# voxel-tracer/ag-pathtracer

Measured on AMD Instinct MI355X. Metric: Mrays/sec (primary+secondary) at 1080p/64spp, higher is better.
Workload: dtype f32; 1 GPU; BASELINE configs[2]: Sponza-class closed atrium, 258672 tris / 37 primitives / 35 Disney materials, 1920x1080, 64 spp, PathTracer MaxDepth=5, NEE+MIS; triangles=258672, spp=64

## Files before the change

### ag-pathtracer_amd/csrc/agpt_api.hip

```cpp
#include <hip/hip_runtime.h>

#include <algorithm>
#include <cmath>
#include <cstdio>
#include <cstdlib>
#include <cstring>
#include <memory>
#include <string>
#include <vector>

#include "../../include/agpt.h"
#include "agpt_adaptive.h"
#include "agpt_bvh_device.h"
#include "agpt_denoise.h"
#include "agpt_host_scene.hpp"
#include "agpt_kernels.h"
#include "agpt_update.h"

#ifndef AGPT_FAST_STACK
#define AGPT_FAST_STACK 23
#endif
#ifndef AGPT_FAST_BLOCKS_PER_CU
#define AGPT_FAST_BLOCKS_PER_CU 5
#endif


namespace {

thread_local std::string g_error;

int fail(int code, const std::string& msg) {
    g_error = msg;
    return code;
}

}
namespace agpt {
int report_error(int code, const std::string& msg) { return fail(code, msg); }
}
namespace {

#define HIP_TRY(expr)                                                                                   \
    do {                                                                                                \
        hipError_t e_ = (expr);                                                                         \
        if (e_ != hipSuccess)                                                                           \
            return fail(AGPT_ERR_DEVICE, std::string(#expr) + ": " + hipGetErrorString(e_));           \
    } while (0)
// ... 28 lines not shown
    }
    void release() {
        if (p) (void)hipFree(p);
        p = nullptr;
        n = 0;
    }
};

}

#define AGPT_POOL_BUFFERS(X)                                                                                                  \
    X(float4, ext_o) X(float4, ext_d) X(float4, sh_o) X(float4, sh_d) X(float4, mis_o) X(float4, mis_d) X(float4, beta4)      \
    X(float4, L4) X(float4, fac4) X(float4, c1) X(float4, c2) X(DevHit, hit) X(DevHit, mis_hit) X(uint32_t, occluded)          \
    X(uint32_t, mis_ok)

struct agpt_ctx {
    int device = 0;
    hipStream_t stream = nullptr;
    int num_cus = 256;
    hipEvent_t ev[4] = {nullptr, nullptr, nullptr, nullptr};
    hipStream_t aux_stream[2] = {nullptr, nullptr};
    hipEvent_t aux_ev[3] = {nullptr, nullptr, nullptr};
    int multi_stream = 0;
    size_t pool_paths = 0;
#define X(T, name) DevBuf<T> name;
    AGPT_POOL_BUFFERS(X)
#undef X
    DevBuf<uint32_t> q[2][AGPT_NQUEUES];
    DevBuf<uint32_t> qcounts;
    DevBuf<uint32_t> work;
    DevBuf<DevCounters> counters;
    uint32_t* host_pinned = nullptr;
    int blocks_per_cu = 4;
    int shade_blocks_per_cu = 8;
    int fast_blocks_per_cu = AGPT_FAST_BLOCKS_PER_CU;
    DevBuf<uint32_t> spill;
    DevBuf<unsigned long long> cand_mask;
    DevBuf<uint32_t> cand_chunks;
    DevBuf<uint32_t> adapt_masks, adapt_blocks, adapt_list, adapt_words;
    DevBuf<float4> denoise_state;
    int refill = AGPT_REFILL;
    int refill_any = AGPT_REFILL_ANY;
    bool mis_closest = false;
    bool force_generic = false;
    std::vector<hipEvent_t> tev;
    size_t tev_used = 0;
// ... 70 lines not shown
}

static int trace_grid(const agpt_ctx* c) { return c->num_cus * c->blocks_per_cu; }
static int fast_grid(const agpt_ctx* c) { return c->num_cus * c->fast_blocks_per_cu; }

static bool use_fast_trace(const agpt_ctx* c, const DevScene& sc, int count) {
    return count != 1 && sc.n_prims <= 64 * AGPT_MAX_CHUNKS && !c->force_generic;
}

#define AGPT_SMALL_BATCH (48ull << 20)

struct TraceLaunch {
    hipStream_t stream;
    const uint32_t* queue;
    const uint32_t* count_ptr;
    uint32_t count_imm;
    uint32_t* work_head;
    const float4 *ro, *rd;
    DevHit* hits;
    uint32_t* occ;
    int count;
    bool small_batch;
    bool recast;
};

template <int MODE, bool COUNT, bool SPILL, bool PEEK>
static void launch_trace_fast(agpt_ctx* c, const DevScene& sc, const TraceLaunch& t) {
    const dim3 block(AGPT_BLOCK), g(fast_grid(c));
    const int refill = MODE == 0 ? c->refill : c->refill_any;
    if (sc.n_prims <= 64) {
        float4* ro_w = MODE == 0 && t.recast ? const_cast<float4*>(t.ro) : nullptr;
        float4* rd_w = MODE == 0 && t.recast ? const_cast<float4*>(t.rd) : nullptr;
        hipLaunchKernelGGL((k_trace_fast<MODE, AGPT_FAST_STACK, false, COUNT, SPILL, PEEK>), g, block, 0, t.stream, sc, t.queue, t.count_ptr,
                           t.count_imm, t.work_head, t.ro, t.rd, t.hits, t.occ, c->counters.p, refill, 0u, c->spill.p,
                           (const unsigned long long*)nullptr, (const uint32_t*)nullptr, ro_w, rd_w, (const float4*)c->beta4.p, c->L4.p);
        return;
    }
    const uint32_t stride = (uint32_t)c->pool_paths;
    if (c->cand_chunks.n < c->pool_paths || c->cand_mask.n < (size_t)((sc.n_prims + 63) / 64) * c->pool_paths) {
        c->note(hipErrorOutOfMemory);
        return;
    }
    hipLaunchKernelGGL((k_candidates<MODE>), dim3(c->num_cus * 8), block, 0, t.stream, sc, t.queue, t.count_ptr, t.count_imm, t.ro, t.rd,
                       c->cand_mask.p, c->cand_chunks.p, stride);
    hipLaunchKernelGGL((k_trace_fast<MODE, AGPT_FAST_STACK, true, COUNT, SPILL, PEEK>), g, block, 0, t.stream, sc, t.queue, t.count_ptr,
                       t.count_imm, t.work_head, t.ro, t.rd, t.hits, t.occ, c->counters.p, refill, stride, c->spill.p,
                       (const unsigned long long*)c->cand_mask.p, (const uint32_t*)c->cand_chunks.p, (float4*)nullptr, (float4*)nullptr,
                       (const float4*)nullptr, (float4*)nullptr);
}

template <bool ANY, bool COUNT, int DEPTH>
static void launch_trace_generic(agpt_ctx* c, int grid, const DevScene& sc, const TraceLaunch& t) {
    hipLaunchKernelGGL((k_trace<ANY, COUNT, DEPTH>), dim3(grid), dim3(AGPT_BLOCK), 0, t.stream, sc, t.queue, t.count_ptr, t.count_imm,
                       t.work_head, t.ro, t.rd, t.hits, t.occ, c->counters.p);
}

template <int MODE>
static void launch_trace(agpt_ctx* c, const DevScene& sc, const TraceLaunch& t) {
// ... 58 lines not shown

extern "C" {

const char* agpt_last_error(void) { return g_error.c_str(); }
int agpt_version(void) { return 1; }

int agpt_init(int device, agpt_ctx** out) {
    if (!out) return fail(AGPT_ERR_INVALID, "agpt_init: out is NULL");
    int n = 0;
    hipError_t e = hipGetDeviceCount(&n);
    if (e != hipSuccess || n == 0)
        return fail(AGPT_ERR_DEVICE, "agpt_init: no HIP device (the MI355X path has no CPU fallback)");
    if (device < 0 || device >= n) return fail(AGPT_ERR_INVALID, "agpt_init: bad device index");
    HIP_TRY(hipSetDevice(device));
    std::unique_ptr<agpt_ctx> c(new agpt_ctx());
    c->device = device;
    hipDeviceProp_t prop;
    HIP_TRY(hipGetDeviceProperties(&prop, device));
    c->num_cus = prop.multiProcessorCount > 0 ? prop.multiProcessorCount : 256;
    for (auto& ev : c->ev) HIP_TRY(hipEventCreate(&ev));
    for (auto& st : c->aux_stream) HIP_TRY(hipStreamCreateWithFlags(&st, hipStreamNonBlocking));
    for (auto& ev : c->aux_ev) HIP_TRY(hipEventCreateWithFlags(&ev, hipEventDisableTiming));
    if (const char* ms = getenv("AGPT_MULTI_STREAM")) c->multi_stream = atoi(ms);
    HIP_TRY(hipHostMalloc((void**)&c->host_pinned, 2 * AGPT_NQUEUES * AGPT_QSTRIDE * sizeof(uint32_t)));
    const char* fg = getenv("AGPT_FORCE_GENERIC");
    c->force_generic = fg && fg[0] == '1';
    if (const char* mc = getenv("AGPT_MIS_CLOSEST")) c->mis_closest = mc[0] == '1';
    if (const char* bp = getenv("AGPT_BLOCKS_PER_CU")) c->fast_blocks_per_cu = std::max(1, atoi(bp));
    if (const char* sb = getenv("AGPT_SHADE_BLOCKS_PER_CU")) c->shade_blocks_per_cu = std::min(64, std::max(1, atoi(sb)));
    if (const char* rf = getenv("AGPT_REFILL")) c->refill = std::min(64, std::max(1, atoi(rf)));
    if (const char* rf = getenv("AGPT_REFILL_ANY")) c->refill_any = std::min(64, std::max(1, atoi(rf)));
    *out = c.release();
    return AGPT_OK;
}

int agpt_set_stream(agpt_ctx* c, void* s) {
    if (!c) return fail(AGPT_ERR_INVALID, "agpt_set_stream: ctx is NULL");
    c->stream = (hipStream_t)s;
    return AGPT_OK;
}

void agpt_destroy(agpt_ctx* c) {
    if (!c) return;
    (void)hipSetDevice(c->device);
    (void)hipDeviceSynchronize();
    if (c->host_pinned) (void)hipHostFree(c->host_pinned);
    for (auto& ev : c->tev) (void)hipEventDestroy(ev);
    for (auto& ev : c->ev)
        if (ev) (void)hipEventDestroy(ev);
    for (auto& ev : c->aux_ev)
        if (ev) (void)hipEventDestroy(ev);
    for (auto& st : c->aux_stream)
        if (st) (void)hipStreamDestroy(st);
    delete c;
}

int agpt_scene_create(agpt_ctx* c, agpt_scene** out) {
    if (!c || !out) return fail(AGPT_ERR_INVALID, "agpt_scene_create: NULL argument");
    agpt_scene* s = new agpt_scene();
    s->ctx = c;
    *out = s;
    return AGPT_OK;
}

void agpt_scene_destroy(agpt_scene* s) {
    if (!s) return;
    (void)hipSetDevice(s->ctx->device);
    (void)hipDeviceSynchronize();
    delete s;
}

int agpt_scene_add_material(agpt_scene* s, int type, const float color[3], float roughness, float metallic) {
    if (!s || !color) return fail(AGPT_ERR_INVALID, "agpt_scene_add_material: NULL argument");
    if (type < AGPT_MAT_DISNEY || type > AGPT_MAT_DIFFUSE_ONLY) return fail(AGPT_ERR_INVALID, "unknown material type");
// ... 636 lines not shown
    HIP_TRY(hipStreamSynchronize(c->stream));
    return AGPT_OK;
}

#define X(T, name) +sizeof(T)
constexpr size_t AGPT_BYTES_PER_PATH = (0 AGPT_POOL_BUFFERS(X)) + 2 * AGPT_NQUEUES * sizeof(uint32_t);
#undef X
static_assert(AGPT_BYTES_PER_PATH == 256, "11 float4 arrays + 2 hit arrays (16 B) + 2 flag words + 10 queue words");
static size_t candidate_bytes_per_path(int n_prims) { return n_prims > 64 ? 4 + 8 * (size_t)((n_prims + 63) / 64) : 0; }
static int ensure_pool(agpt_ctx* c, size_t paths, int n_prims) {
    int rc;
    paths = std::max(paths, c->pool_paths);
    if (n_prims > 64) {
        if ((rc = c->cand_chunks.ensure(paths))) return rc;
        if ((rc = c->cand_mask.ensure(paths * (size_t)((n_prims + 63) / 64)))) return rc;
    }
#define X(T, name) \
    if ((rc = c->name.ensure(paths))) return rc;
    AGPT_POOL_BUFFERS(X)
#undef X
    for (int i = 0; i < 2; i++)
        for (int j = 0; j < AGPT_NQUEUES; j++)
            if ((rc = c->q[i][j].ensure(paths))) return rc;
    if ((rc = c->qcounts.ensure(2 * AGPT_NQUEUES * AGPT_QSTRIDE))) return rc;
    if ((rc = c->work.ensure(4096))) return rc;
    if ((rc = c->counters.ensure(1))) return rc;
    c->pool_paths = paths;
    return AGPT_OK;
}

static int fit_pool(agpt_ctx* c, const agpt_scene* s, size_t unit, uint64_t& count) {
    if (unit * (size_t)count > c->pool_paths) {
        size_t free_b = 0, total_b = 0;
        if (hipMemGetInfo(&free_b, &total_b) == hipSuccess) {
            const size_t per_path = AGPT_BYTES_PER_PATH + candidate_bytes_per_path(s->dev.n_prims);
            const size_t avail = free_b + c->pool_paths * per_path;
            const size_t fit = (size_t)((double)avail * 0.9) / per_path;
            while (count > 1 && unit * (size_t)count > fit) count = (count + 1) / 2;
        }
    }
    int rc = ensure_pool(c, unit * (size_t)count, s->dev.n_prims);
    while (rc == AGPT_ERR_NOMEM && count > 1) {
        release_pool(c);
        count = (count + 1) / 2;
        rc = ensure_pool(c, unit * (size_t)count, s->dev.n_prims);
    }
    return rc;
// ... 25 lines not shown
    run.count = enable_counters == 2 ? 2 : (enable_counters != 0 ? 1 : 0);
    run.mis_mode = use_fast_trace(c, s->dev, run.count) && !c->mis_closest;
    run.timing = timing;
    run.shade.fast = s->shading_arith == AGPT_SHADING_FAST;
    run.shade.textured = s->textured;
    run.shade.mapped = s->mapped;
    run.shade.sampled = s->sampled;
    run.shade.normal = s->normal;
    run.shade.lds_tables = shade_tables_fit_lds(s->dev);
    run.shade.env = !s->envs.empty();
    c->tev_used = 0;
    c->tev_kind.clear();
    HIP_TRY(hipMemsetAsync(c->counters.p, 0, sizeof(DevCounters), c->stream));
    HIP_TRY(hipEventRecord(c->ev[0], c->stream));
    return AGPT_OK;
}

static void set_wavefront_consts(RenderConsts& rc, const WavefrontRun& run, int max_depth, bool trace_all_rays) {
    rc.max_depth = max_depth;
    rc.mis_mode = run.mis_mode ? 1 : 0;
    rc.answer_rays = (run.mis_mode && !trace_all_rays) ? 1 : 0;
}

static int run_wavefront(agpt_ctx* c, agpt_scene* s, const RenderConsts& rcn, WavefrontRun& run) {
    const int count = run.count;
    const PathBuffers& pb = run.pb;
    Queues* const q = run.q;
    const int shade_grid = c->num_cus * c->shade_blocks_per_cu;
    const bool small_batch = (unsigned long long)rcn.NP * (unsigned long long)rcn.S < AGPT_SMALL_BATCH;
    const bool recast = !getenv("AGPT_NO_RECAST");
    const bool side = (c->multi_stream == 2 || (c->multi_stream == 1 && small_batch)) && use_fast_trace(c, s->dev, count) &&
                      s->dev.max_depth <= AGPT_FAST_STACK && s->dev.n_prims <= 64;
    const hipStream_t main_stream = c->stream, mis_stream = side ? c->aux_stream[0] : main_stream,
                      shadow_stream = side ? c->aux_stream[1] : main_stream;
    int cur = 0;
    const int planned = rcn.max_depth + 2;
    for (int it = 0;; it++) {
        if (it >= planned) {
            uint32_t* slot = c->host_pinned + (it & 1) * (AGPT_NQUEUES * AGPT_QSTRIDE);
            HIP_TRY(hipMemcpyAsync(slot, q[cur].counts, (4 * AGPT_QSTRIDE + 1) * sizeof(uint32_t), hipMemcpyDeviceToHost, main_stream));
            HIP_TRY(hipEventRecord(c->ev[2 + (it & 1)], main_stream));
            if (it > planned) {
                const uint32_t* seen = c->host_pinned + ((it - 1) & 1) * (AGPT_NQUEUES * AGPT_QSTRIDE);
                HIP_TRY(hipEventSynchronize(c->ev[2 + ((it - 1) & 1)]));
                if (seen[0] == 0 && seen[4 * AGPT_QSTRIDE] == 0) break;
            }
            if (it > 4096) return fail(AGPT_ERR_LIMIT, "agpt: path did not terminate");
        }
        const int nxt = cur ^ 1;
        HIP_TRY(hipMemsetAsync(q[nxt].counts, 0, AGPT_NQUEUES * AGPT_QSTRIDE * sizeof(uint32_t), main_stream));
        HIP_TRY(hipMemsetAsync(c->work.p, 0, 4 * AGPT_FRONTIERS * AGPT_QSTRIDE * sizeof(uint32_t), main_stream));
        uint32_t* const heads[4] = {c->work.p, c->work.p + AGPT_FRONTIERS * AGPT_QSTRIDE, c->work.p + 2 * AGPT_FRONTIERS * AGPT_QSTRIDE,
                                    c->work.p + 3 * AGPT_FRONTIERS * AGPT_QSTRIDE};
        const TraceLaunch ext{main_stream, q[cur].ext, &QCOUNT(q[cur], 1), 0, heads[0], pb.ext_o, pb.ext_d, pb.hit, nullptr,
                              count, small_batch, recast};
        const TraceLaunch mis{mis_stream, q[cur].mis, &QCOUNT(q[cur], 2), 0, heads[1], pb.mis_o, pb.mis_d,
                              run.mis_mode ? nullptr : pb.mis_hit, run.mis_mode ? pb.mis_ok : nullptr, count, small_batch, false};
        const TraceLaunch shadow{shadow_stream, q[cur].shadow, &QCOUNT(q[cur], 3), 0, heads[2], pb.sh_o, pb.sh_d, nullptr, pb.occluded,
                                 count, small_batch, false};
        auto trace_ext = [&]() { launch_trace_timed<0>(c, run.timing, 0, s->dev, ext); };
        auto trace_mis = [&]() {
            if (run.mis_mode) launch_trace_timed<2>(c, run.timing, 1, s->dev, mis);
            else launch_trace_timed<0>(c, run.timing, 1, s->dev, mis);
        };
        auto trace_shadow = [&]() { launch_trace_timed<1>(c, run.timing, 2, s->dev, shadow); };
        if (side) {
            HIP_TRY(hipEventRecord(c->aux_ev[0], main_stream));
            HIP_TRY(hipStreamWaitEvent(mis_stream, c->aux_ev[0], 0));
            HIP_TRY(hipStreamWaitEvent(shadow_stream, c->aux_ev[0], 0));
            trace_mis();
            HIP_TRY(hipEventRecord(c->aux_ev[1], mis_stream));
            trace_shadow();
            HIP_TRY(hipEventRecord(c->aux_ev[2], shadow_stream));
            trace_ext();
            HIP_TRY(hipStreamWaitEvent(main_stream, c->aux_ev[1], 0));
            HIP_TRY(hipStreamWaitEvent(main_stream, c->aux_ev[2], 0));
        } else {
            trace_ext();
            trace_mis();
            trace_shadow();
        }
        agpt::launch_shading(main_stream, run.shade, shade_grid, c->num_cus * 8, s->dev, rcn, pb, q[cur], q[nxt], c->counters.p, heads[3]);
        cur = nxt;
        run.iterations++;
        run.launches += 3;
    }
    return AGPT_OK;
}

static void read_counters(const DevCounters& d, agpt_stats* st) {
    st->closest_rays = d.closest_rays;
    st->anyhit_rays = d.anyhit_rays;
    st->interior_visits = d.interior;
    st->root_tests = d.roots;
    st->tri_tests = d.tris;
    st->shaded_vertices = d.shaded;
    st->outliers = d.outliers;
    st->samples = d.samples;
    st->answered_rays = d.answered;
}

static int end_wavefront(agpt_ctx* c) {
    HIP_TRY(hipEventRecord(c->ev[1], c->stream));
    HIP_TRY(hipGetLastError());
    HIP_TRY(c->take_deferred());
    return AGPT_OK;
}

static int fill_stats(agpt_ctx* c, const WavefrontRun& run, uint64_t samples, agpt_stats* stats) {
    if (!stats) return AGPT_OK;
// ... 211 lines not shown
int agpt_render(agpt_scene* s, const agpt_render_params* rp, float* accum_dev, agpt_stats* stats) {
    if (!s || !rp || !accum_dev) return fail(AGPT_ERR_INVALID, "agpt_render: NULL argument");
    if (!s->committed || !s->has_camera) return fail(AGPT_ERR_INVALID, "agpt_render: scene not committed or camera not set");
    int rc;
    if ((rc = check_tile("agpt_render", rp)) || (rc = check_depth("agpt_render", rp->max_depth))) return rc;
    if (rp->spp_count < 0) return fail(AGPT_ERR_INVALID, "agpt_render: bad sample range");
    agpt_ctx* c = s->ctx;
    HIP_TRY(hipSetDevice(c->device));
    uint32_t rows;
    if ((rc = tile_rows("agpt_render", rp, rows))) return rc;
    if (rows == 0) return AGPT_OK;
    const uint32_t NP = (uint32_t)rp->w * rows;
    uint64_t batch = std::min<uint64_t>(samples_per_batch(rp, NP), (uint64_t)std::max(1, rp->spp_count));
    if ((uint64_t)NP * batch > 0x7FFFFFFFull) return fail(AGPT_ERR_LIMIT, "agpt_render: batch too large");
    if ((rc = fit_pool(c, s, NP, batch))) return rc;
    const int S = (int)batch;
    s->dev.cam = s->cam;

    WavefrontRun run;
    if ((rc = begin_wavefront(c, s, rp->enable_counters, rp->enable_timing != 0 && stats != nullptr, run))) return rc;
    RenderConsts rcn = tile_consts(rp, NP);
    rcn.seed_base = rp->seed_base;
    set_wavefront_consts(rcn, run, rp->max_depth, rp->trace_all_rays != 0);
    for (int s0 = rp->spp_begin; s0 < rp->spp_begin + rp->spp_count; s0 += S) {
        rcn.s0 = s0;
        rcn.S = std::min(S, rp->spp_begin + rp->spp_count - s0);
        const uint32_t total = NP * (uint32_t)rcn.S;
        hipLaunchKernelGGL(k_generate, dim3((total + AGPT_BLOCK - 1) / AGPT_BLOCK), dim3(AGPT_BLOCK), 0, c->stream, s->dev, rcn, run.pb,
                           run.q[0]);
        if ((rc = run_wavefront(c, s, rcn, run))) return rc;
        hipLaunchKernelGGL(k_accumulate, dim3((NP + AGPT_BLOCK - 1) / AGPT_BLOCK), dim3(AGPT_BLOCK), 0, c->stream, rcn, run.pb,
                           (float4*)accum_dev, c->counters.p);
    }
    if ((rc = end_wavefront(c))) return rc;
    return fill_stats(c, run, (uint64_t)NP * (uint64_t)rp->spp_count, stats);
}

int agpt_render_adaptive(agpt_scene* s, const agpt_render_params* rp, const agpt_adaptive_params* ap, float* accum_dev,
                         float* moment2_dev, agpt_stats* stats, agpt_adaptive_stats* astats) {
    if (!s || !rp || !ap || !accum_dev || !moment2_dev) return fail(AGPT_ERR_INVALID, "agpt_render_adaptive: NULL argument");
    if (!s->committed || !s->has_camera) return fail(AGPT_ERR_INVALID, "agpt_render_adaptive: scene not committed or camera not set");
    int rc;
    if ((rc = check_tile("agpt_render_adaptive", rp)) || (rc = check_depth("agpt_render_adaptive", rp->max_depth))) return rc;
    if (rp->spp_begin != 0 || rp->spp_count != 0)
        return fail(AGPT_ERR_INVALID, "agpt_render_adaptive: spp_begin and spp_count must be 0 (the counts are in accum.w)");
    const int step = ap->step_spp, min_spp = ap->min_spp, max_spp = ap->max_spp;
    if (step < 1 || min_spp < 2 || min_spp > max_spp || max_spp > (1 << 24) || min_spp % step != 0 || max_spp % step != 0 ||
        !(ap->abs_floor >= 0.f) || ap->rel_error != ap->rel_error)
        return fail(AGPT_ERR_INVALID, "agpt_render_adaptive: need 1 <= step_spp, 2 <= min_spp <= max_spp <= 2^24, both multiples of "
                                      "step_spp, abs_floor >= 0, rel_error not NaN");
    if (astats) std::memset(astats, 0, sizeof(*astats));
    agpt_ctx* c = s->ctx;
    HIP_TRY(hipSetDevice(c->device));
    uint32_t rows;
    if ((rc = tile_rows("agpt_render_adaptive", rp, rows))) return rc;
// ... 496 lines not shown
```

### ag-pathtracer_amd/csrc/agpt_kernels.h

```cpp
#pragma once

#include "agpt_shade.h"
#include "agpt_trace.h"

#include "agpt_wavefront.h"

template <bool ANY, bool COUNT, int DEPTH>
__global__ void __launch_bounds__(AGPT_BLOCK)
k_trace(DevScene sc, const uint32_t* __restrict__ queue, const uint32_t* __restrict__ count_ptr, uint32_t count_imm,
        uint32_t* __restrict__ work_head, const float4* __restrict__ ray_o, const float4* __restrict__ ray_d,
        DevHit* __restrict__ hits, uint32_t* __restrict__ occluded, DevCounters* __restrict__ counters) {
    __shared__ uint32_t s_stack[DEPTH * AGPT_BLOCK];
    uint32_t* stack = s_stack + threadIdx.x;
    const int lane = threadIdx.x & 63;
    const uint32_t count = count_ptr ? *count_ptr : count_imm;
    TraceCounters cnt;
    cnt.interior = 0;
    cnt.tris = 0;
    cnt.roots = 0;
    cnt.last_mesh = 0;
    for (;;) {
        uint32_t base = 0;
        if (lane == 0) base = atomicAdd(work_head, (uint32_t)AGPT_CHUNK);
        base = __shfl(base, 0);
// ... 20 lines not shown
            atomicAdd(&counters->interior, (unsigned long long)cnt.interior);
            atomicAdd(&counters->tris, (unsigned long long)cnt.tris);
            atomicAdd(&counters->roots, (unsigned long long)cnt.roots);
        }
    }
    if (threadIdx.x == 0 && blockIdx.x == 0) {
        if (ANY)
            atomicAdd(&counters->anyhit_rays, (unsigned long long)count);
        else
            atomicAdd(&counters->closest_rays, (unsigned long long)count);
    }
}

#define AGPT_REFILL 20
#define AGPT_REFILL_ANY 40
#define AGPT_RING 128

#ifndef AGPT_TRACE_WAVES
#define AGPT_TRACE_WAVES 1
#endif
template <int MODE, int DEPTH, bool LIST, bool COUNT, bool SPILL, bool PEEK>
__global__ void __launch_bounds__(AGPT_BLOCK, AGPT_TRACE_WAVES)
k_trace_fast(DevScene sc, const uint32_t* __restrict__ queue, const uint32_t* __restrict__ count_ptr, uint32_t count_imm,
             uint32_t* __restrict__ work_head, const float4* __restrict__ ray_o, const float4* __restrict__ ray_d,
             DevHit* __restrict__ hits, uint32_t* __restrict__ occluded, DevCounters* __restrict__ counters, int refill,
             uint32_t cand_stride, uint32_t* __restrict__ spill, const unsigned long long* __restrict__ cand_mask,
             const uint32_t* __restrict__ cand_chunks, float4* ray_o_w, float4* ray_d_w, const float4* path_beta4, float4* path_L4) {
    constexpr bool ANY = MODE != 0;
    constexpr bool MIS = MODE == 2;
    constexpr int BLOCK = AGPT_BLOCK;
    constexpr bool PRIM_LDS = !LIST;
    __shared__ uint32_t s_stack[DEPTH * BLOCK];
    __shared__ float4 s_prim[PRIM_LDS ? 2 * 64 : 2];
    uint32_t* stack = s_stack + threadIdx.x;
    uint32_t* spill_col = SPILL ? spill + (size_t)blockIdx.x * BLOCK + threadIdx.x : nullptr;
    const size_t spill_stride = (size_t)gridDim.x * BLOCK;
    auto stack_push = [&](int k, uint32_t v) {
        if (!SPILL || k < DEPTH)
            stack[k * BLOCK] = v;
        else
            spill_col[(size_t)(k - DEPTH) * spill_stride] = v;
    };
    auto stack_at = [&](int k) -> uint32_t {
        if (!SPILL || k < DEPTH) return stack[k * BLOCK];
        return spill_col[(size_t)(k - DEPTH) * spill_stride];
    };
    const int lane = threadIdx.x & 63;
// ... 820 lines not shown
```

### ag-pathtracer_amd/csrc/agpt_shade_kernels.h

```cpp
#pragma once

#include "agpt_shade.h"
#include "agpt_trace.h"
#include "agpt_wavefront.h"

#ifndef AGPT_SHADE_TEXTURED
#define AGPT_SHADE_TEXTURED 0
#endif
#if AGPT_SHADE_TEXTURED == 4 && AGPT_SHADE_FAST
#define AGPT_SHADE_KNAME(n) n##_normal_fast
#elif AGPT_SHADE_TEXTURED == 4
#define AGPT_SHADE_KNAME(n) n##_normal
#elif AGPT_SHADE_TEXTURED == 3 && AGPT_SHADE_FAST
#define AGPT_SHADE_KNAME(n) n##_sampled_fast
#elif AGPT_SHADE_TEXTURED == 3
#define AGPT_SHADE_KNAME(n) n##_sampled
#elif AGPT_SHADE_TEXTURED == 2 && AGPT_SHADE_FAST
#define AGPT_SHADE_KNAME(n) n##_mapped_fast
#elif AGPT_SHADE_TEXTURED == 2
#define AGPT_SHADE_KNAME(n) n##_mapped
#elif AGPT_SHADE_TEXTURED && AGPT_SHADE_FAST
#define AGPT_SHADE_KNAME(n) n##_textured_fast
#elif AGPT_SHADE_TEXTURED
#define AGPT_SHADE_KNAME(n) n##_textured
// ... 411 lines not shown
    l4.x = L.x; l4.y = L.y; l4.z = L.z; l4.w = __uint_as_float(rng);
    pb.L4[pid] = l4;
    SCK(6);
    return bits;
}

#ifndef SHADE_GRAB
#define SHADE_GRAB 2
#endif
#ifndef SHADE_U
#define SHADE_U 4
#endif

#ifndef AGPT_SHADE_WAVES
#define AGPT_SHADE_WAVES 3
#endif
#define AGPT_SHADE_LDS_PRIMS 256
#define AGPT_SHADE_LDS_MATERIALS 128
#define AGPT_SHADE_LDS_LIGHTS 64
template <bool LDS_TABLES, bool ENV>
__global__ void __launch_bounds__(AGPT_BLOCK, AGPT_SHADE_WAVES)
AGPT_SHADE_KNAME(k_shade)(DevScene sc_in, RenderConsts rc, PathBuffers pb, Queues qin, Queues qout, DevCounters* __restrict__ counters,
        uint32_t* __restrict__ tile_heads) {
    __shared__ DevPrim s_tab_prims[LDS_TABLES ? AGPT_SHADE_LDS_PRIMS : 1];
    __shared__ DevMaterial s_tab_materials[LDS_TABLES ? AGPT_SHADE_LDS_MATERIALS : 1];
    __shared__ DevLight s_tab_lights[LDS_TABLES ? AGPT_SHADE_LDS_LIGHTS : 1];
#if AGPT_SHADE_TEXTURED
    constexpr int n_tab_halves = AGPT_SHADE_TEXTURED >= 2 ? 2 : 1;
    __shared__ int32_t s_tab_material_texture[LDS_TABLES ? n_tab_halves * AGPT_SHADE_LDS_MATERIALS : 1];
#endif
    if (blockIdx.x * (AGPT_BLOCK / 64) * 64u * SHADE_U >= QCOUNT(qin, 0) && blockIdx.x > 0) return;
    DevScene sc = sc_in;
    if (LDS_TABLES) {
        auto copy_words = [&](void* dst, const void* src, int n_bytes) {
            uint32_t* d = (uint32_t*)dst;
            const uint32_t* g = (const uint32_t*)src;
            for (int i = threadIdx.x; i < n_bytes / 4; i += AGPT_BLOCK) d[i] = g[i];
        };
        copy_words(s_tab_prims, sc_in.prims, sc_in.n_prims * (int)sizeof(DevPrim));
        copy_words(s_tab_materials, sc_in.materials, sc_in.n_materials * (int)sizeof(DevMaterial));
        copy_words(s_tab_lights, sc_in.lights, sc_in.n_lights * (int)sizeof(DevLight));
        sc.prims = s_tab_prims;
        sc.materials = s_tab_materials;
        sc.lights = s_tab_lights;
#if AGPT_SHADE_TEXTURED
        copy_words(s_tab_material_texture, sc_in.material_texture, n_tab_halves * sc_in.n_materials * (int)sizeof(int32_t));
        sc.material_texture = s_tab_material_texture;
#endif
        __syncthreads();
    }
    __shared__ uint32_t s_pid[SHADE_U][AGPT_BLOCK];
    __shared__ uint32_t s_bits[SHADE_U][AGPT_BLOCK];
    const uint32_t n_active = QCOUNT(qin, 0);
    const int tid = threadIdx.x, lane = tid & 63;
    const unsigned long long lt_mask = (1ull << lane) - 1ull;
    uint32_t shaded = 0, mis_answered = 0;
#ifdef AGPT_SHADE_CLOCK
    unsigned long long sck_acc[8] = {0, 0, 0, 0, 0, 0, 0, 0};
    unsigned long long sck_last = __builtin_amdgcn_s_memtime();
    const unsigned long long sck_begin = sck_last;
#endif
    const uint32_t wtile = 64u * SHADE_U;
    const uint32_t n_wtiles = (n_active + wtile - 1) / wtile;
    uint32_t seg = blockIdx.x & (AGPT_FRONTIERS - 1u), segs_left = AGPT_FRONTIERS;
    const uint32_t seg_tiles = (n_wtiles + AGPT_FRONTIERS - 1u) / AGPT_FRONTIERS;
    uint32_t t_next = 0, t_end = 0;
    auto next_tile = [&](uint32_t& t) -> bool {
        if (t_next < t_end) {
            t = t_next++;
            return true;
// ... 95 lines not shown
        const float4 c1_4 = pb.c1[pid], c2_4 = pb.c2[pid];
        const uint32_t flags = __float_as_uint(b4.w);
        const v3 Ld = pending_light_sample(sc, rc, pb, pid, flags, was_occluded, was_mis_ok, c1_4, c2_4, f4);
        const float lightPdf = sh_rcp(sc.n_lights);
        const v3 L = V3(l4.x, l4.y, l4.z) + V3(b4.x, b4.y, b4.z) * sh_div3(Ld, lightPdf);
        l4.x = L.x; l4.y = L.y; l4.z = L.z;
        pb.L4[pid] = l4;
    }
}
#endif

namespace agpt {
using ShadeLaunch = void(hipStream_t stream, int grid, bool lds_tables, bool env, const DevScene& sc, const RenderConsts& rc,
                         const PathBuffers& pb, const Queues& qin, const Queues& qout, DevCounters* counters, uint32_t* tile_heads);
using ResolveLaunch = void(hipStream_t stream, int grid, const DevScene& sc, const RenderConsts& rc, const PathBuffers& pb, const Queues& qin);
ShadeLaunch launch_shade, launch_shade_fast, launch_shade_textured, launch_shade_textured_fast, launch_shade_mapped, launch_shade_mapped_fast,
    launch_shade_sampled, launch_shade_sampled_fast, launch_shade_normal, launch_shade_normal_fast;
ResolveLaunch launch_resolve_pending, launch_resolve_pending_fast;

void AGPT_SHADE_KNAME(launch_shade)(hipStream_t stream, int grid, bool lds_tables, bool env, const DevScene& sc, const RenderConsts& rc,
                                    const PathBuffers& pb, const Queues& qin, const Queues& qout, DevCounters* counters,
                                    uint32_t* tile_heads) {
    const dim3 g(grid), b(AGPT_BLOCK);
    if (lds_tables && env)
        hipLaunchKernelGGL((AGPT_SHADE_KNAME(k_shade)<true, true>), g, b, 0, stream, sc, rc, pb, qin, qout, counters, tile_heads);
    else if (lds_tables)
        hipLaunchKernelGGL((AGPT_SHADE_KNAME(k_shade)<true, false>), g, b, 0, stream, sc, rc, pb, qin, qout, counters, tile_heads);
    else if (env)
        hipLaunchKernelGGL((AGPT_SHADE_KNAME(k_shade)<false, true>), g, b, 0, stream, sc, rc, pb, qin, qout, counters, tile_heads);
    else
        hipLaunchKernelGGL((AGPT_SHADE_KNAME(k_shade)<false, false>), g, b, 0, stream, sc, rc, pb, qin, qout, counters, tile_heads);
}
#if !AGPT_SHADE_TEXTURED
void AGPT_SHADE_KNAME(launch_resolve_pending)(hipStream_t stream, int grid, const DevScene& sc, const RenderConsts& rc,
                                              const PathBuffers& pb, const Queues& qin) {
    hipLaunchKernelGGL(AGPT_SHADE_KNAME(k_resolve_pending), dim3(grid), dim3(AGPT_BLOCK), 0, stream, sc, rc, pb, qin);
}
#endif
}
```

### ag-pathtracer_amd/csrc/agpt_wavefront.h

```cpp
#pragma once

#include "agpt_math.h"
#include "agpt_scene.h"

#define AGPT_BLOCK 256
#define AGPT_CHUNK 64

#define PF_BOUNCE_MASK 0xFFu
#define PF_SPECULAR 0x100u
#define PF_DEAD 0x200u
#define PF_PEND_C1 0x400u
#define PF_PEND_C2 0x800u
#define PF_PENDING 0x1000u

struct PathBuffers {
    float4 *ext_o, *ext_d;
    float4 *sh_o, *sh_d;
    float4 *mis_o, *mis_d;
    DevHit *hit, *mis_hit;
    uint32_t* occluded;
    uint32_t* mis_ok;
    float4* beta4;
    float4* L4;
    float4* fac4;
// ... 2 lines not shown

#define AGPT_QSTRIDE 32
#ifndef AGPT_FRONTIERS
#define AGPT_FRONTIERS 8u
#endif
struct Queues {
    uint32_t *active, *ext, *mis, *shadow;
    uint32_t* resolve;
    uint32_t* counts;
};
#define AGPT_NQUEUES 5
#define QCOUNT(q, i) ((q).counts[(i) * AGPT_QSTRIDE])

struct RenderConsts {
    int32_t W, H, x0, y0, w, h;
    int32_t s0, S;
    uint32_t seed_base;
    int32_t max_depth;
    int32_t accum_pitch, accum_row0;
    uint32_t NP;
    int32_t il_block, il_world, il_rank;
    int32_t mis_mode;
    int32_t answer_rays;
};

__device__ __forceinline__ uint32_t sample_group(int32_t S) {
    const uint32_t low = (uint32_t)S & (0u - (uint32_t)S);
    return low < 64u ? low : 64u;
}

__device__ __forceinline__ void pixel_of(const RenderConsts& rc, uint32_t p, int& x, int& y, size_t& accum_index) {
    const uint32_t w = (uint32_t)rc.w, n_rows = rc.NP / w;
    uint32_t row, col;
    if (((w | n_rows) & 7u) == 0u) {
        const uint32_t blk = p >> 6, inner = p & 63u, per_row = w >> 3;
        const uint32_t brow = blk / per_row;
        row = brow * 8u + (inner >> 3);
        col = (blk - brow * per_row) * 8u + (inner & 7u);
    } else {
        row = p / w;
        col = p - row * w;
    }
    x = rc.x0 + (int)col;
    if (rc.il_block == 0) {
        y = rc.y0 + (int)row;
        accum_index = (size_t)((rc.H - 1 - y) - rc.accum_row0) * (size_t)rc.accum_pitch + (size_t)x;
    } else {
        const int j = (int)row / rc.il_block, within = (int)row % rc.il_block;
        const int yb = (j * rc.il_world + rc.il_rank) * rc.il_block;
        const int hb = min(rc.il_block, rc.H - yb);
        y = yb + within;
        accum_index = (size_t)(j * rc.il_block + (hb - 1 - within)) * (size_t)rc.accum_pitch + (size_t)x;
    }
}

struct DevCounters {
    unsigned long long closest_rays, anyhit_rays, interior, tris, shaded, outliers, samples, roots, answered;
#if defined(AGPT_TRACE_STATS) || defined(AGPT_SHADE_CLOCK)
    unsigned long long dbg[64];
#endif
};
#ifdef AGPT_TRACE_STATS
#define TS(...) __VA_ARGS__
#else
#define TS(...)
// ... 39 lines not shown
```

Measured before the change: 4164 Mrays/s.

## Split the image into two halves and pipeline trace/shade across two streams

Refactors the wavefront loop into a Pipeline abstraction and adds an optional mode that splits each sample batch into two row halves on separate streams. One half's shading can overlap the other's tracing, with a reduced trace grid and shade grid while both are active. It also switches the shade kernel's LDS tables to dynamic shared memory sized to the actual scene, which may improve occupancy. Overlap is off by default (AGPT_OVERLAP_DEFAULT 0) and the trace guard requires n_prims <= 64, which this 37-primitive scene meets.

```diff
diff --git a/ag-pathtracer_amd/csrc/agpt_api.hip b/ag-pathtracer_amd/csrc/agpt_api.hip
--- a/ag-pathtracer_amd/csrc/agpt_api.hip
+++ b/ag-pathtracer_amd/csrc/agpt_api.hip
@@ -23,6 +23,9 @@
 #ifndef AGPT_FAST_BLOCKS_PER_CU
 #define AGPT_FAST_BLOCKS_PER_CU 5
 #endif
+#ifndef AGPT_OVERLAP_DEFAULT
+#define AGPT_OVERLAP_DEFAULT 0
+#endif
 
 
 namespace {
@@ -97,6 +100,10 @@
     hipStream_t aux_stream[2] = {nullptr, nullptr};
     hipEvent_t aux_ev[3] = {nullptr, nullptr, nullptr};
     int multi_stream = 0;
+    int overlap = AGPT_OVERLAP_DEFAULT;
+    int overlap_trace_blocks = 4, overlap_shade_blocks = 1;
+    hipEvent_t half_ev[2][3] = {};
+    hipEvent_t fork_ev = nullptr, join_ev = nullptr;
     size_t pool_paths = 0;
 #define X(T, name) DevBuf<T> name;
     AGPT_POOL_BUFFERS(X)
@@ -213,18 +220,21 @@
     int count;
     bool small_batch;
     bool recast;
+    const float4* beta4 = nullptr;
+    float4* L4 = nullptr;
+    int blocks_per_cu = 0;
 };
 
 template <int MODE, bool COUNT, bool SPILL, bool PEEK>
 static void launch_trace_fast(agpt_ctx* c, const DevScene& sc, const TraceLaunch& t) {
-    const dim3 block(AGPT_BLOCK), g(fast_grid(c));
+    const dim3 block(AGPT_BLOCK), g(t.blocks_per_cu > 0 ? c->num_cus * t.blocks_per_cu : fast_grid(c));
     const int refill = MODE == 0 ? c->refill : c->refill_any;
     if (sc.n_prims <= 64) {
         float4* ro_w = MODE == 0 && t.recast ? const_cast<float4*>(t.ro) : nullptr;
         float4* rd_w = MODE == 0 && t.recast ? const_cast<float4*>(t.rd) : nullptr;
         hipLaunchKernelGGL((k_trace_fast<MODE, AGPT_FAST_STACK, false, COUNT, SPILL, PEEK>), g, block, 0, t.stream, sc, t.queue, t.count_ptr,
                            t.count_imm, t.work_head, t.ro, t.rd, t.hits, t.occ, c->counters.p, refill, 0u, c->spill.p,
-                           (const unsigned long long*)nullptr, (const uint32_t*)nullptr, ro_w, rd_w, (const float4*)c->beta4.p, c->L4.p);
+                           (const unsigned long long*)nullptr, (const uint32_t*)nullptr, ro_w, rd_w, t.beta4, t.L4);
         return;
     }
     const uint32_t stride = (uint32_t)c->pool_paths;
@@ -329,7 +339,14 @@
     for (auto& st : c->aux_stream) HIP_TRY(hipStreamCreateWithFlags(&st, hipStreamNonBlocking));
     for (auto& ev : c->aux_ev) HIP_TRY(hipEventCreateWithFlags(&ev, hipEventDisableTiming));
     if (const char* ms = getenv("AGPT_MULTI_STREAM")) c->multi_stream = atoi(ms);
-    HIP_TRY(hipHostMalloc((void**)&c->host_pinned, 2 * AGPT_NQUEUES * AGPT_QSTRIDE * sizeof(uint32_t)));
+    for (auto& half : c->half_ev)
+        for (auto& ev : half) HIP_TRY(hipEventCreateWithFlags(&ev, hipEventDisableTiming));
+    HIP_TRY(hipEventCreateWithFlags(&c->fork_ev, hipEventDisableTiming));
+    HIP_TRY(hipEventCreateWithFlags(&c->join_ev, hipEventDisableTiming));
+    if (const char* ov = getenv("AGPT_OVERLAP")) c->overlap = std::min(2, std::max(0, atoi(ov)));
+    if (const char* tb = getenv("AGPT_OVERLAP_TRACE_BLOCKS")) c->overlap_trace_blocks = std::min(8, std::max(1, atoi(tb)));
+    if (const char* sb = getenv("AGPT_OVERLAP_SHADE_BLOCKS")) c->overlap_shade_blocks = std::min(64, std::max(1, atoi(sb)));
+    HIP_TRY(hipHostMalloc((void**)&c->host_pinned, 4 * AGPT_NQUEUES * AGPT_QSTRIDE * sizeof(uint32_t)));
     const char* fg = getenv("AGPT_FORCE_GENERIC");
     c->force_generic = fg && fg[0] == '1';
     if (const char* mc = getenv("AGPT_MIS_CLOSEST")) c->mis_closest = mc[0] == '1';
@@ -357,6 +374,11 @@
         if (ev) (void)hipEventDestroy(ev);
     for (auto& ev : c->aux_ev)
         if (ev) (void)hipEventDestroy(ev);
+    for (auto& half : c->half_ev)
+        for (auto& ev : half)
+            if (ev) (void)hipEventDestroy(ev);
+    if (c->fork_ev) (void)hipEventDestroy(c->fork_ev);
+    if (c->join_ev) (void)hipEventDestroy(c->join_ev);
     for (auto& st : c->aux_stream)
         if (st) (void)hipStreamDestroy(st);
     delete c;
@@ -1039,7 +1061,7 @@
     for (int i = 0; i < 2; i++)
         for (int j = 0; j < AGPT_NQUEUES; j++)
             if ((rc = c->q[i][j].ensure(paths))) return rc;
-    if ((rc = c->qcounts.ensure(2 * AGPT_NQUEUES * AGPT_QSTRIDE))) return rc;
+    if ((rc = c->qcounts.ensure(2 * 2 * AGPT_NQUEUES * AGPT_QSTRIDE))) return rc;
     if ((rc = c->work.ensure(4096))) return rc;
     if ((rc = c->counters.ensure(1))) return rc;
     c->pool_paths = paths;
@@ -1111,70 +1133,157 @@
     rc.answer_rays = (run.mis_mode && !trace_all_rays) ? 1 : 0;
 }
 
+struct Pipeline {
+    PathBuffers pb;
+    Queues q[2];
+    RenderConsts rc;
+    hipStream_t stream;
+    uint32_t* work;
+    uint32_t* pinned;
+    hipEvent_t check_ev[2];
+    hipEvent_t traced;
+    int cur = 0, it = 0;
+    bool done = false;
+};
+
+static Pipeline make_pipeline(agpt_ctx* c, const WavefrontRun& run, const RenderConsts& rc, int half, size_t first_path, hipStream_t stream) {
+    Pipeline p;
+#define X(T, name) p.pb.name = run.pb.name + first_path;
+    AGPT_POOL_BUFFERS(X)
+#undef X
+    for (int i = 0; i < 2; i++) {
+        const Queues& q = run.q[i];
+        p.q[i] = Queues{q.active + first_path, q.ext + first_path, q.mis + first_path, q.shadow + first_path, q.resolve + first_path,
+                        q.counts + 2 * AGPT_NQUEUES * AGPT_QSTRIDE * half};
+    }
+    p.rc = rc;
+    p.stream = stream;
+    p.work = c->work.p + 4 * AGPT_FRONTIERS * AGPT_QSTRIDE * half;
+    p.pinned = c->host_pinned + 2 * AGPT_NQUEUES * AGPT_QSTRIDE * half;
+    p.check_ev[0] = half ? c->half_ev[1][1] : c->ev[2];
+    p.check_ev[1] = half ? c->half_ev[1][2] : c->ev[3];
+    p.traced = c->half_ev[half][0];
+    return p;
+}
+
+struct LaunchShape {
+    bool side;
+    int trace_blocks_per_cu;
+    int shade_grid;
+};
+
+static int pipeline_check(agpt_ctx* c, Pipeline& p) {
+    const int it = p.it, planned = p.rc.max_depth + 2;
+    if (it < planned) return AGPT_OK;
+    uint32_t* slot = p.pinned + (it & 1) * (AGPT_NQUEUES * AGPT_QSTRIDE);
+    HIP_TRY(hipMemcpyAsync(slot, p.q[p.cur].counts, (4 * AGPT_QSTRIDE + 1) * sizeof(uint32_t), hipMemcpyDeviceToHost, p.stream));
+    HIP_TRY(hipEventRecord(p.check_ev[it & 1], p.stream));
+    if (it > planned) {
+        const uint32_t* seen = p.pinned + ((it - 1) & 1) * (AGPT_NQUEUES * AGPT_QSTRIDE);
+        HIP_TRY(hipEventSynchronize(p.check_ev[(it - 1) & 1]));
+        if (seen[0] == 0 && seen[4 * AGPT_QSTRIDE] == 0) p.done = true;
+    }
+    if (!p.done && it > 4096) return fail(AGPT_ERR_LIMIT, "agpt: path did not terminate");
+    return AGPT_OK;
+}
+
+static int pipeline_trace(agpt_ctx* c, agpt_scene* s, WavefrontRun& run, Pipeline& p, const LaunchShape& shape) {
+    const int count = run.count;
+    const PathBuffers& pb = p.pb;
+    Queues* const q = p.q;
+    const int cur = p.cur, nxt = cur ^ 1;
+    const bool small_batch = (unsigned long long)p.rc.NP * (unsigned long long)p.rc.S < AGPT_SMALL_BATCH;
+    const bool recast = !getenv("AGPT_NO_RECAST");
+    const hipStream_t main_stream = p.stream, mis_stream = shape.side ? c->aux_stream[0] : main_stream,
+                      shadow_stream = shape.side ? c->aux_stream[1] : main_stream;
+    HIP_TRY(hipMemsetAsync(q[nxt].counts, 0, AGPT_NQUEUES * AGPT_QSTRIDE * sizeof(uint32_t), main_stream));
+    HIP_TRY(hipMemsetAsync(p.work, 0, 4 * AGPT_FRONTIERS * AGPT_QSTRIDE * sizeof(uint32_t), main_stream));
+    uint32_t* const heads[3] = {p.work, p.work + AGPT_FRONTIERS * AGPT_QSTRIDE, p.work + 2 * AGPT_FRONTIERS * AGPT_QSTRIDE};
+    const TraceLaunch ext{main_stream, q[cur].ext, &QCOUNT(q[cur], 1), 0, heads[0], pb.ext_o, pb.ext_d, pb.hit, nullptr,
+                          count, small_batch, recast, pb.beta4, pb.L4, shape.trace_blocks_per_cu};
+    const TraceLaunch mis{mis_stream, q[cur].mis, &QCOUNT(q[cur], 2), 0, heads[1], pb.mis_o, pb.mis_d,
+                          run.mis_mode ? nullptr : pb.mis_hit, run.mis_mode ? pb.mis_ok : nullptr, count, small_batch, false,
+                          nullptr, nullptr, shape.trace_blocks_per_cu};
+    const TraceLaunch shadow{shadow_stream, q[cur].shadow, &QCOUNT(q[cur], 3), 0, heads[2], pb.sh_o, pb.sh_d, nullptr, pb.occluded,
+                             count, small_batch, false, nullptr, nullptr, shape.trace_blocks_per_cu};
+    auto trace_ext = [&]() { launch_trace_timed<0>(c, run.timing, 0, s->dev, ext); };
+    auto trace_mis = [&]() {
+        if (run.mis_mode) launch_trace_timed<2>(c, run.timing, 1, s->dev, mis);
+        else launch_trace_timed<0>(c, run.timing, 1, s->dev, mis);
+    };
+    auto trace_shadow = [&]() { launch_trace_timed<1>(c, run.timing, 2, s->dev, shadow); };
+    if (shape.side) {
+        HIP_TRY(hipEventRecord(c->aux_ev[0], main_stream));
+        HIP_TRY(hipStreamWaitEvent(mis_stream, c->aux_ev[0], 0));
+        HIP_TRY(hipStreamWaitEvent(shadow_stream, c->aux_ev[0], 0));
+        trace_mis();
+        HIP_TRY(hipEventRecord(c->aux_ev[1], mis_stream));
+        trace_shadow();
+        HIP_TRY(hipEventRecord(c->aux_ev[2], shadow_stream));
+        trace_ext();
+        HIP_TRY(hipStreamWaitEvent(main_stream, c->aux_ev[1], 0));
+        HIP_TRY(hipStreamWaitEvent(main_stream, c->aux_ev[2], 0));
+    } else {
+        trace_ext();
+        trace_mis();
+        trace_shadow();
+    }
+    return AGPT_OK;
+}
+
+static void pipeline_shade(agpt_ctx* c, agpt_scene* s, WavefrontRun& run, Pipeline& p, const LaunchShape& shape) {
+    const int nxt = p.cur ^ 1;
+    agpt::launch_shading(p.stream, run.shade, shape.shade_grid, c->num_cus * 8, s->dev, p.rc, p.pb, p.q[p.cur], p.q[nxt], c->counters.p,
+                         p.work + 3 * AGPT_FRONTIERS * AGPT_QSTRIDE);
+    p.cur = nxt;
+    p.it++;
+    run.launches += 3;
+}
+
 static int run_wavefront(agpt_ctx* c, agpt_scene* s, const RenderConsts& rcn, WavefrontRun& run) {
-    const int count = run.count;
-    const PathBuffers& pb = run.pb;
-    Queues* const q = run.q;
-    const int shade_grid = c->num_cus * c->shade_blocks_per_cu;
+    Pipeline p = make_pipeline(c, run, rcn, 0, 0, c->stream);
     const bool small_batch = (unsigned long long)rcn.NP * (unsigned long long)rcn.S < AGPT_SMALL_BATCH;
-    const bool recast = !getenv("AGPT_NO_RECAST");
-    const bool side = (c->multi_stream == 2 || (c->multi_stream == 1 && small_batch)) && use_fast_trace(c, s->dev, count) &&
+    const bool side = (c->multi_stream == 2 || (c->multi_stream == 1 && small_batch)) && use_fast_trace(c, s->dev, run.count) &&
                       s->dev.max_depth <= AGPT_FAST_STACK && s->dev.n_prims <= 64;
-    const hipStream_t main_stream = c->stream, mis_stream = side ? c->aux_stream[0] : main_stream,
-                      shadow_stream = side ? c->aux_stream[1] : main_stream;
-    int cur = 0;
-    const int planned = rcn.max_depth + 2;
-    for (int it = 0;; it++) {
-        if (it >= planned) {
-            uint32_t* slot = c->host_pinned + (it & 1) * (AGPT_NQUEUES * AGPT_QSTRIDE);
-            HIP_TRY(hipMemcpyAsync(slot, q[cur].counts, (4 * AGPT_QSTRIDE + 1) * sizeof(uint32_t), hipMemcpyDeviceToHost, main_stream));
-            HIP_TRY(hipEventRecord(c->ev[2 + (it & 1)], main_stream));
-            if (it > planned) {
-                const uint32_t* seen = c->host_pinned + ((it - 1) & 1) * (AGPT_NQUEUES * AGPT_QSTRIDE);
-                HIP_TRY(hipEventSynchronize(c->ev[2 + ((it - 1) & 1)]));
-                if (seen[0] == 0 && seen[4 * AGPT_QSTRIDE] == 0) break;
-            }
-            if (it > 4096) return fail(AGPT_ERR_LIMIT, "agpt: path did not terminate");
+    const LaunchShape shape{side, 0, c->num_cus * c->shade_blocks_per_cu};
+    for (;;) {
+        if (const int rc = pipeline_check(c, p)) return rc;
+        if (p.done) break;
+        if (const int rc = pipeline_trace(c, s, run, p, shape)) return rc;
+        pipeline_shade(c, s, run, p, shape);
+    }
+    run.iterations += (uint64_t)p.it;
+    return AGPT_OK;
+}
+
+static int run_wavefront_halves(agpt_ctx* c, agpt_scene* s, WavefrontRun& run, Pipeline (&P)[2]) {
+    const LaunchShape beside{false, c->overlap_trace_blocks, c->num_cus * c->overlap_shade_blocks},
+                      alone{false, 0, c->num_cus * c->shade_blocks_per_cu};
+    bool traced[2] = {false, false};
+    while (!P[0].done || !P[1].done) {
+        for (int h = 0; h < 2; h++) {
+            Pipeline &p = P[h], &other = P[h ^ 1];
+            if (p.done) continue;
+            if (const int rc = pipeline_check(c, p)) return rc;
+            if (p.done) continue;
+            const LaunchShape& shape = other.done ? alone : beside;
+            if (traced[h ^ 1]) HIP_TRY(hipStreamWaitEvent(p.stream, other.traced, 0));
+            if (const int rc = pipeline_trace(c, s, run, p, shape)) return rc;
+            HIP_TRY(hipEventRecord(p.traced, p.stream));
+            traced[h] = true;
+            pipeline_shade(c, s, run, p, shape);
         }
-        const int nxt = cur ^ 1;
-        HIP_TRY(hipMemsetAsync(q[nxt].counts, 0, AGPT_NQUEUES * AGPT_QSTRIDE * sizeof(uint32_t), main_stream));
-        HIP_TRY(hipMemsetAsync(c->work.p, 0, 4 * AGPT_FRONTIERS * AGPT_QSTRIDE * sizeof(uint32_t), main_stream));
-        uint32_t* const heads[4] = {c->work.p, c->work.p + AGPT_FRONTIERS * AGPT_QSTRIDE, c->work.p + 2 * AGPT_FRONTIERS * AGPT_QSTRIDE,
-                                    c->work.p + 3 * AGPT_FRONTIERS * AGPT_QSTRIDE};
-        const TraceLaunch ext{main_stream, q[cur].ext, &QCOUNT(q[cur], 1), 0, heads[0], pb.ext_o, pb.ext_d, pb.hit, nullptr,
-                              count, small_batch, recast};
-        const TraceLaunch mis{mis_stream, q[cur].mis, &QCOUNT(q[cur], 2), 0, heads[1], pb.mis_o, pb.mis_d,
-                              run.mis_mode ? nullptr : pb.mis_hit, run.mis_mode ? pb.mis_ok : nullptr, count, small_batch, false};
-        const TraceLaunch shadow{shadow_stream, q[cur].shadow, &QCOUNT(q[cur], 3), 0, heads[2], pb.sh_o, pb.sh_d, nullptr, pb.occluded,
-                                 count, small_batch, false};
-        auto trace_ext = [&]() { launch_trace_timed<0>(c, run.timing, 0, s->dev, ext); };
-        auto trace_mis = [&]() {
-            if (run.mis_mode) launch_trace_timed<2>(c, run.timing, 1, s->dev, mis);
-            else launch_trace_timed<0>(c, run.timing, 1, s->dev, mis);
-        };
-        auto trace_shadow = [&]() { launch_trace_timed<1>(c, run.timing, 2, s->dev, shadow); };
-        if (side) {
-            HIP_TRY(hipEventRecord(c->aux_ev[0], main_stream));
-            HIP_TRY(hipStreamWaitEvent(mis_stream, c->aux_ev[0], 0));
-            HIP_TRY(hipStreamWaitEvent(shadow_stream, c->aux_ev[0], 0));
-            trace_mis();
-            HIP_TRY(hipEventRecord(c->aux_ev[1], mis_stream));
-            trace_shadow();
-            HIP_TRY(hipEventRecord(c->aux_ev[2], shadow_stream));
-            trace_ext();
-            HIP_TRY(hipStreamWaitEvent(main_stream, c->aux_ev[1], 0));
-            HIP_TRY(hipStreamWaitEvent(main_stream, c->aux_ev[2], 0));
-        } else {
-            trace_ext();
-            trace_mis();
-            trace_shadow();
-        }
-        agpt::launch_shading(main_stream, run.shade, shade_grid, c->num_cus * 8, s->dev, rcn, pb, q[cur], q[nxt], c->counters.p, heads[3]);
-        cur = nxt;
-        run.iterations++;
-        run.launches += 3;
-    }
-    return AGPT_OK;
+    }
+    run.iterations += (uint64_t)std::max(P[0].it, P[1].it);
+    return AGPT_OK;
+}
+
+static uint32_t overlap_rows(const agpt_ctx* c, const agpt_scene* s, const WavefrontRun& run, uint32_t w, uint32_t rows, int S) {
+    if (c->overlap == 0 || !use_fast_trace(c, s->dev, run.count) || s->dev.max_depth > AGPT_FAST_STACK || s->dev.n_prims > 64) return 0;
+    const uint32_t first = (rows / 2 + 7) / 8 * 8;
+    if (first >= rows) return 0;
+    if (c->overlap == 1 && (run.count != 0 || (unsigned long long)w * (rows - first) * (unsigned long long)S < AGPT_SMALL_BATCH)) return 0;
+    return first;
 }
 
 static void read_counters(const DevCounters& d, agpt_stats* st) {
@@ -1432,15 +1541,40 @@
     RenderConsts rcn = tile_consts(rp, NP);
     rcn.seed_base = rp->seed_base;
     set_wavefront_consts(rcn, run, rp->max_depth, rp->trace_all_rays != 0);
+    auto generate = [&](const Pipeline& p) {
+        const uint32_t total = p.rc.NP * (uint32_t)p.rc.S;
+        hipLaunchKernelGGL(k_generate, dim3((total + AGPT_BLOCK - 1) / AGPT_BLOCK), dim3(AGPT_BLOCK), 0, p.stream, s->dev, p.rc, p.pb, p.q[0]);
+    };
+    auto accumulate = [&](const Pipeline& p) {
+        hipLaunchKernelGGL(k_accumulate, dim3((p.rc.NP + AGPT_BLOCK - 1) / AGPT_BLOCK), dim3(AGPT_BLOCK), 0, p.stream, p.rc, p.pb,
+                           (float4*)accum_dev, c->counters.p);
+    };
     for (int s0 = rp->spp_begin; s0 < rp->spp_begin + rp->spp_count; s0 += S) {
         rcn.s0 = s0;
         rcn.S = std::min(S, rp->spp_begin + rp->spp_count - s0);
-        const uint32_t total = NP * (uint32_t)rcn.S;
-        hipLaunchKernelGGL(k_generate, dim3((total + AGPT_BLOCK - 1) / AGPT_BLOCK), dim3(AGPT_BLOCK), 0, c->stream, s->dev, rcn, run.pb,
-                           run.q[0]);
-        if ((rc = run_wavefront(c, s, rcn, run))) return rc;
-        hipLaunchKernelGGL(k_accumulate, dim3((NP + AGPT_BLOCK - 1) / AGPT_BLOCK), dim3(AGPT_BLOCK), 0, c->stream, rcn, run.pb,
-                           (float4*)accum_dev, c->counters.p);
+        const uint32_t first_rows = overlap_rows(c, s, run, (uint32_t)rp->w, rows, rcn.S);
+        if (first_rows == 0) {
+            Pipeline p = make_pipeline(c, run, rcn, 0, 0, c->stream);
+            generate(p);
+            if ((rc = run_wavefront(c, s, rcn, run))) return rc;
+            accumulate(p);
+            continue;
+        }
+        RenderConsts rch[2] = {rcn, rcn};
+        rch[0].NP = (uint32_t)rp->w * first_rows;
+        rch[1].NP = NP - rch[0].NP;
+        rch[1].row0 = (int32_t)first_rows;
+        Pipeline P[2] = {make_pipeline(c, run, rch[0], 0, 0, c->stream),
+                         make_pipeline(c, run, rch[1], 1, (size_t)rch[0].NP * (size_t)S, c->aux_stream[0])};
+        HIP_TRY(hipEventRecord(c->fork_ev, c->stream));
+        HIP_TRY(hipStreamWaitEvent(P[1].stream, c->fork_ev, 0));
+        generate(P[0]);
+        generate(P[1]);
+        if ((rc = run_wavefront_halves(c, s, run, P))) return rc;
+        accumulate(P[0]);
+        accumulate(P[1]);
+        HIP_TRY(hipEventRecord(c->join_ev, P[1].stream));
+        HIP_TRY(hipStreamWaitEvent(c->stream, c->join_ev, 0));
     }
     if ((rc = end_wavefront(c))) return rc;
     return fill_stats(c, run, (uint64_t)NP * (uint64_t)rp->spp_count, stats);
diff --git a/ag-pathtracer_amd/csrc/agpt_kernels.h b/ag-pathtracer_amd/csrc/agpt_kernels.h
--- a/ag-pathtracer_amd/csrc/agpt_kernels.h
+++ b/ag-pathtracer_amd/csrc/agpt_kernels.h
@@ -66,7 +66,7 @@
 template <int MODE, int DEPTH, bool LIST, bool COUNT, bool SPILL, bool PEEK>
 __global__ void __launch_bounds__(AGPT_BLOCK, AGPT_TRACE_WAVES)
 k_trace_fast(DevScene sc, const uint32_t* __restrict__ queue, const uint32_t* __restrict__ count_ptr, uint32_t count_imm,
-             uint32_t* __restrict__ work_head, const float4* __restrict__ ray_o, const float4* __restrict__ ray_d,
+             uint32_t* __restrict__ work_head, const float4* ray_o, const float4* ray_d,
              DevHit* __restrict__ hits, uint32_t* __restrict__ occluded, DevCounters* __restrict__ counters, int refill,
              uint32_t cand_stride, uint32_t* __restrict__ spill, const unsigned long long* __restrict__ cand_mask,
              const uint32_t* __restrict__ cand_chunks, float4* ray_o_w, float4* ray_d_w, const float4* path_beta4, float4* path_L4) {
diff --git a/ag-pathtracer_amd/csrc/agpt_shade_kernels.h b/ag-pathtracer_amd/csrc/agpt_shade_kernels.h
--- a/ag-pathtracer_amd/csrc/agpt_shade_kernels.h
+++ b/ag-pathtracer_amd/csrc/agpt_shade_kernels.h
@@ -457,30 +457,29 @@
 __global__ void __launch_bounds__(AGPT_BLOCK, AGPT_SHADE_WAVES)
 AGPT_SHADE_KNAME(k_shade)(DevScene sc_in, RenderConsts rc, PathBuffers pb, Queues qin, Queues qout, DevCounters* __restrict__ counters,
         uint32_t* __restrict__ tile_heads) {
-    __shared__ DevPrim s_tab_prims[LDS_TABLES ? AGPT_SHADE_LDS_PRIMS : 1];
-    __shared__ DevMaterial s_tab_materials[LDS_TABLES ? AGPT_SHADE_LDS_MATERIALS : 1];
-    __shared__ DevLight s_tab_lights[LDS_TABLES ? AGPT_SHADE_LDS_LIGHTS : 1];
-#if AGPT_SHADE_TEXTURED
-    constexpr int n_tab_halves = AGPT_SHADE_TEXTURED >= 2 ? 2 : 1;
-    __shared__ int32_t s_tab_material_texture[LDS_TABLES ? n_tab_halves * AGPT_SHADE_LDS_MATERIALS : 1];
-#endif
+    extern __shared__ uint32_t s_tables[];
     if (blockIdx.x * (AGPT_BLOCK / 64) * 64u * SHADE_U >= QCOUNT(qin, 0) && blockIdx.x > 0) return;
     DevScene sc = sc_in;
     if (LDS_TABLES) {
-        auto copy_words = [&](void* dst, const void* src, int n_bytes) {
-            uint32_t* d = (uint32_t*)dst;
+        auto copy_words = [&](uint32_t* d, const void* src, int n_words) {
             const uint32_t* g = (const uint32_t*)src;
-            for (int i = threadIdx.x; i < n_bytes / 4; i += AGPT_BLOCK) d[i] = g[i];
+            for (int i = threadIdx.x; i < n_words; i += AGPT_BLOCK) d[i] = g[i];
         };
-        copy_words(s_tab_prims, sc_in.prims, sc_in.n_prims * (int)sizeof(DevPrim));
-        copy_words(s_tab_materials, sc_in.materials, sc_in.n_materials * (int)sizeof(DevMaterial));
-        copy_words(s_tab_lights, sc_in.lights, sc_in.n_lights * (int)sizeof(DevLight));
-        sc.prims = s_tab_prims;
-        sc.materials = s_tab_materials;
-        sc.lights = s_tab_lights;
+        constexpr int prim_words = (int)sizeof(DevPrim) / 4, material_words = (int)sizeof(DevMaterial) / 4, light_words = (int)sizeof(DevLight) / 4;
+        uint32_t* const tab_prims = s_tables;
+        uint32_t* const tab_materials = tab_prims + sc_in.n_prims * prim_words;
+        uint32_t* const tab_lights = tab_materials + sc_in.n_materials * material_words;
+        copy_words(tab_prims, sc_in.prims, sc_in.n_prims * prim_words);
+        copy_words(tab_materials, sc_in.materials, sc_in.n_materials * material_words);
+        copy_words(tab_lights, sc_in.lights, sc_in.n_lights * light_words);
+        sc.prims = (const DevPrim*)tab_prims;
+        sc.materials = (const DevMaterial*)tab_materials;
+        sc.lights = (const DevLight*)tab_lights;
 #if AGPT_SHADE_TEXTURED
-        copy_words(s_tab_material_texture, sc_in.material_texture, n_tab_halves * sc_in.n_materials * (int)sizeof(int32_t));
-        sc.material_texture = s_tab_material_texture;
+        constexpr int n_tab_halves = AGPT_SHADE_TEXTURED >= 2 ? 2 : 1;
+        uint32_t* const tab_material_texture = tab_lights + sc_in.n_lights * light_words;
+        copy_words(tab_material_texture, sc_in.material_texture, n_tab_halves * sc_in.n_materials);
+        sc.material_texture = (const int32_t*)tab_material_texture;
 #endif
         __syncthreads();
     }
@@ -622,10 +621,13 @@
                                     const PathBuffers& pb, const Queues& qin, const Queues& qout, DevCounters* counters,
                                     uint32_t* tile_heads) {
     const dim3 g(grid), b(AGPT_BLOCK);
+    const size_t lds = !lds_tables ? 0
+                                   : sc.n_prims * sizeof(DevPrim) + sc.n_materials * sizeof(DevMaterial) + sc.n_lights * sizeof(DevLight) +
+                                         (AGPT_SHADE_TEXTURED >= 2 ? 2 : AGPT_SHADE_TEXTURED ? 1 : 0) * sc.n_materials * sizeof(int32_t);
     if (lds_tables && env)
-        hipLaunchKernelGGL((AGPT_SHADE_KNAME(k_shade)<true, true>), g, b, 0, stream, sc, rc, pb, qin, qout, counters, tile_heads);
+        hipLaunchKernelGGL((AGPT_SHADE_KNAME(k_shade)<true, true>), g, b, lds, stream, sc, rc, pb, qin, qout, counters, tile_heads);
     else if (lds_tables)
-        hipLaunchKernelGGL((AGPT_SHADE_KNAME(k_shade)<true, false>), g, b, 0, stream, sc, rc, pb, qin, qout, counters, tile_heads);
+        hipLaunchKernelGGL((AGPT_SHADE_KNAME(k_shade)<true, false>), g, b, lds, stream, sc, rc, pb, qin, qout, counters, tile_heads);
     else if (env)
         hipLaunchKernelGGL((AGPT_SHADE_KNAME(k_shade)<false, true>), g, b, 0, stream, sc, rc, pb, qin, qout, counters, tile_heads);
     else
diff --git a/ag-pathtracer_amd/csrc/agpt_wavefront.h b/ag-pathtracer_amd/csrc/agpt_wavefront.h
--- a/ag-pathtracer_amd/csrc/agpt_wavefront.h
+++ b/ag-pathtracer_amd/csrc/agpt_wavefront.h
@@ -48,6 +48,7 @@
     int32_t il_block, il_world, il_rank;
     int32_t mis_mode;
     int32_t answer_rays;
+    int32_t row0;
 };
 
 __device__ __forceinline__ uint32_t sample_group(int32_t S) {
@@ -67,6 +68,7 @@
         row = p / w;
         col = p - row * w;
     }
+    row += (uint32_t)rc.row0;
     x = rc.x0 + (int)col;
     if (rc.il_block == 0) {
         y = rc.y0 + (int)row;
```

New measurement: 4181 Mrays/s (median of 6 runs). About the same (+0.4%).
